# sapienta-ai/general-motion-retargeting

Measured on AMD Instinct MI355X. Metric: retargeted frames/sec (whole node) + max joint-angle err vs CPU ref, G1 29-DoF, higher is better.
Workload: dtype f64

## Files before the change

### __graft_entry__.py

```python
import os
import sys

ROOT = os.path.dirname(os.path.abspath(__file__))
if ROOT not in sys.path:
    sys.path.insert(0, ROOT)


def build() -> None:
    from general_motion_retargeting_amd import build as hip_build
    lib_path = hip_build.build(force=True)
    assert os.path.exists(lib_path)
    from oracle import oracle
    oracle.build(force=True)
    for p in list(hip_build.build_probe(force=True).values()) + list(hip_build.build_jlinv_probe(force=True).values()):
        assert os.path.exists(p)
    import general_motion_retargeting_amd as pkg
    from general_motion_retargeting_amd import _lib
    from general_motion_retargeting_amd.ik_config import pack_model, pack_taskset
    L = _lib.lib()
    for sym in _lib.EXPORTED_SYMBOLS:
        assert hasattr(L, sym), sym
    g = pkg.GeneralMotionRetargeting("smplx", "unitree_g1")
    oracle.check_abi(pack_model(g.model), pack_taskset(g.model, g._tables))


def smoke() -> None:
    import numpy as np
    import general_motion_retargeting_amd as pkg
    from general_motion_retargeting_amd import _lib, synth
    from oracle import oracle
    _lib.require_gpu()
    info = _lib.lib().gmr_backend_info().decode()
    g = pkg.GeneralMotionRetargeting("smplx", "unitree_g1", actual_human_height=1.75)
    human, q0 = synth.make_streams(g.model, g._tables, 4, 6, seed=0)
    q_hip, ns_hip, st = g.retarget_streams(human)
    q_cpu, ns_cpu, _ = oracle.retarget_streams(g._model_blob, g._taskset_blob, q0, human)
    assert (st == 0).all()
    assert np.array_equal(ns_hip, ns_cpu), "solver iteration counts differ"
    err = float(np.abs(q_hip - q_cpu).max())
    assert err < 1e-9, err
    for t, hd in enumerate(synth.streams_to_dicts(g._tables, human[0])):
        q = g.retarget(hd)
        assert np.abs(q - q_cpu[0, t]).max() < 1e-9
    km = pkg.KinematicsModel(g.xml_file)
    qq = q_hip[0]
    bp, br = km.forward_kinematics(qq[:, :3], qq[:, [4, 5, 6, 3]], qq[:, 7:])
    obp, obr = oracle.fk_f32(km._tree, qq[:, :3], qq[:, [4, 5, 6, 3]], qq[:, 7:])
    assert np.abs(bp - obp).max() < 5e-6 and np.abs(br - obr).max() < 5e-6
    print(f"smoke ok on {info}: max |q_hip - q_oracle| = {err:.2e}, solves/frame = {ns_hip.sum() / ns_hip[..., 0].size:.2f}")


if __name__ == "__main__":
    build()
    if len(sys.argv) > 1 and sys.argv[1] == "smoke":
        smoke()
```

### general_motion_retargeting_amd/build.py

```python
from __future__ import annotations

import hashlib
import os
import shutil
import subprocess
import sys

HERE = os.path.dirname(os.path.abspath(__file__))
CSRC = os.path.join(HERE, "csrc")
LIB = os.path.join(HERE, "libgmrhip.so")
OBJ = os.path.join(os.path.dirname(HERE), "build", "obj")
SOURCES = ["gmr_ik.hip", "gmr_ik_wide.hip", "gmr_fk.hip", "gmr_post.hip", "gmr_smplx.hip", "gmr_bvh.hip", "gmr_chunk.hip", "gmr_motion.hip", "gmr_body_state.hip", "gmr_tracker.hip", "gmr_tracker_links.hip", "gmr_tracker_preview.hip", "gmr_tracker_adaptive.hip", "gmr_tracker_anchor.hip", "gmr_tracker_control.hip", "gmr_comm.hip", "gmr_abi.hip"]
HEADERS = ["gmr_ik_wide_item.inc", "gmr_device_math.h", "gmr_ik_layout.h", "gmr_ik_wide_layout.h", "gmr_ik_prof.h", "gmr_ik_tree.h",
           "gmr_fk_tree.h", "gmr_fk_walk.h", "gmr_motion_sample.h", "gmr_philox.h", "gmr_tracker_dev.h", "gmr_link_plan.h", "gmr_handles.h", "gmr_post.h", "gmr_internal.h", "gmr_workspace.h", "../../include/gmr_hip.h", "../../include/gmr_types.h"]
FLAGS = ["-O3", "--offload-arch=gfx950", "-std=c++17", "-fPIC"]
PER_SOURCE_FLAGS = {"gmr_ik_wide.hip": ["-mllvm", "-disable-machine-licm", "-mllvm", "-sink-insts-to-avoid-spills=1"]}


def _hipcc() -> str:
    for c in (os.environ.get("HIPCC"), shutil.which("hipcc"), "/opt/rocm/bin/hipcc"):
        if c and os.path.exists(c):
            return c
    raise RuntimeError("hipcc not found (set HIPCC)")

# ... 11 lines not shown
    per_source = [] if os.environ.get("GMR_BUILD_NO_PER_SOURCE_FLAGS") else PER_SOURCE_FLAGS.get(src, [])
    defines = per_source + list(defines)
    tag = hashlib.sha1(" ".join(FLAGS + defines).encode()).hexdigest()[:10]
    obj = os.path.join(OBJ, f"{os.path.splitext(src)[0]}.{tag}.o")
    deps = [os.path.join(CSRC, src)] + [os.path.join(CSRC, h) for h in HEADERS]
    if force or verbose or not os.path.exists(obj) or any(os.path.getmtime(d) > os.path.getmtime(obj) for d in deps):
        cmd = [_hipcc()] + FLAGS + list(defines) + ["-c", os.path.join(CSRC, src), "-o", obj]
        if verbose:
            cmd.append("-Rpass-analysis=kernel-resource-usage")
        subprocess.check_call(cmd, cwd=CSRC)
    return obj


def _link(objs, out: str) -> str:
    subprocess.check_call([_hipcc(), "--offload-arch=gfx950", "-fPIC", "-shared", "-o", out + ".tmp"] + objs + ["-ldl"])
    os.replace(out + ".tmp", out)
    return out


def build(force: bool = False, verbose: bool = False) -> str:
    if not force and not needs_build():
        return LIB
    return _link([_object(s, [], force, verbose) for s in SOURCES], LIB)


PROBE_SRC = os.path.join(os.path.dirname(HERE), "tests", "hip", "math_probe.hip")
PROBE_LIBS = {"flags": os.path.join(os.path.dirname(PROBE_SRC), "libgmr_math_probe.so"),
              "wide": os.path.join(os.path.dirname(PROBE_SRC), "libgmr_math_probe_wide.so")}


def _build_probe_libs(src: str, libs: dict, force: bool) -> dict:
    deps = [src, os.path.join(CSRC, "gmr_device_math.h"), os.path.abspath(__file__)]
    extra = {"flags": [], "wide": PER_SOURCE_FLAGS["gmr_ik_wide.hip"]}
    for name, out in libs.items():
        if force or not os.path.exists(out) or any(os.path.getmtime(d) > os.path.getmtime(out) for d in deps):
            subprocess.check_call([_hipcc()] + FLAGS + extra[name] + ["-shared", "-o", out + ".tmp", src])
            os.replace(out + ".tmp", out)
    return dict(libs)


def build_probe(force: bool = False) -> dict:
    return _build_probe_libs(PROBE_SRC, PROBE_LIBS, force)


JLINV_PROBE_SRC = os.path.join(os.path.dirname(PROBE_SRC), "jlinv_apply_probe.hip")
JLINV_PROBE_LIBS = {"flags": os.path.join(os.path.dirname(PROBE_SRC), "libgmr_jlinv_apply_probe.so"),
                    "wide": os.path.join(os.path.dirname(PROBE_SRC), "libgmr_jlinv_apply_probe_wide.so")}


def build_jlinv_probe(force: bool = False) -> dict:
    return _build_probe_libs(JLINV_PROBE_SRC, JLINV_PROBE_LIBS, force)


def build_variant(name: str, defines=(), verbose: bool = False) -> str:
    out = os.path.join(HERE, f"libgmrhip_{name}.so")
    return _link([_object(s, list(defines), False, verbose) for s in SOURCES], out)


if __name__ == "__main__":
    if len(sys.argv) > 2 and sys.argv[1] == "--variant":
        print(build_variant(sys.argv[2], sys.argv[3:], verbose=False))
    else:
        print(build(force=True, verbose=True))
```

### general_motion_retargeting_amd/csrc/gmr_device_math.h

```cpp
#pragma once
#include <hip/hip_runtime.h>

namespace gmr {

struct d3 { double x, y, z; };
struct d4 { double w, x, y, z; };

__device__ __forceinline__ d3 operator+(d3 a, d3 b) { return {a.x + b.x, a.y + b.y, a.z + b.z}; }
__device__ __forceinline__ d3 operator-(d3 a, d3 b) { return {a.x - b.x, a.y - b.y, a.z - b.z}; }
__device__ __forceinline__ d3 operator*(double s, d3 a) { return {s * a.x, s * a.y, s * a.z}; }
__device__ __forceinline__ double dot(d3 a, d3 b) { return a.x * b.x + a.y * b.y + a.z * b.z; }
__device__ __forceinline__ d3 cross(d3 a, d3 b) {
  return {a.y * b.z - a.z * b.y, a.z * b.x - a.x * b.z, a.x * b.y - a.y * b.x};
}

__device__ __forceinline__ d4 qmul(d4 a, d4 b) {
  return {a.w * b.w - a.x * b.x - a.y * b.y - a.z * b.z,
          a.w * b.x + a.x * b.w + a.y * b.z - a.z * b.y,
          a.w * b.y - a.x * b.z + a.y * b.w + a.z * b.x,
          a.w * b.z + a.x * b.y - a.y * b.x + a.z * b.w};
}
__device__ __forceinline__ double fast_rsqrt(double x) {
  const double y = __builtin_amdgcn_rsq(x);
  const double e = fma(-x, y * y, 1.0);
// ... 284 lines not shown
  const d3 n = cross(w, rho), m = cross(w, n);
  const double k1 = (c1 + c2) * s;
  const d3 sq = {0.5 * rho.x - k1 * w.x - c2 * m.x, 0.5 * rho.y - k1 * w.y - c2 * m.y, 0.5 * rho.z - k1 * w.z - c2 * m.z};
  const double dq = -2.0 * c1 * s + 2.0 * c4 * s * t2, kw = -2.0 * c4 * s;
  const double da = 1.0 - a * t2;
  const d3 hw = {-0.5 * w.x, -0.5 * w.y, -0.5 * w.z};
  const double awj = a * dot(w, ej);
  const d3 hx = cross(hw, ej);
  const d3 v = {hx.x + awj * w.x + da * ej.x, hx.y + awj * w.y + da * ej.y, hx.z + awj * w.z + da * ej.z};
  const double wv = dot(w, v), rv = dot(rho, v);
  const double kr = c1 * wv, kq = c1 * rv + kw * wv;
  const d3 sx = cross(sq, v);
  const d3 y = {sx.x + kr * rho.x + kq * w.x + dq * v.x, sx.y + kr * rho.y + kq * w.y + dq * v.y, sx.z + kr * rho.z + kq * w.z + dq * v.z};
  const double awy = a * dot(w, y);
  const d3 hy = cross(hw, y);
  Ac[0] = v.x; Ac[1] = v.y; Ac[2] = v.z;
  Bc[0] = -(hy.x + awy * w.x + da * y.x); Bc[1] = -(hy.y + awy * w.y + da * y.y); Bc[2] = -(hy.z + awy * w.z + da * y.z);
}

__device__ __forceinline__ void se3_jlinv_coef5(const double e[6], const double aux[5], double coef[8]) {
  const d3 rho = {e[0], e[1], e[2]}, w = {e[3], e[4], e[5]};
  const double t2 = dot(w, w);
  coef[0] = 0.0; coef[1] = 1.0;
#pragma unroll
  for (int i = 2; i < 8; i++) coef[i] = 0.0;
  if (t2 < 1e-10) return;
  const double a = aux[0];
  double c1, c2, c3;
  if (t2 < 1e-2) {
    c1 = 1.0 / 6.0 - t2 / 120.0 + t2 * t2 / 5040.0 - t2 * t2 * t2 / 362880.0;
    c2 = -1.0 / 24.0 + t2 / 720.0 - t2 * t2 / 40320.0 + t2 * t2 * t2 / 3628800.0;
    c3 = -1.0 / 120.0 + t2 / 5040.0 - t2 * t2 / 362880.0 + t2 * t2 * t2 / 39916800.0;
  } else {
    const double t = aux[3], it = aux[4], sn = aux[1], cs = aux[2];
    const double it2 = it * it;
    c1 = (t - sn) * it2 * it;
    c2 = (1.0 - 0.5 * t2 - cs) * it2 * it2;
    c3 = (t - sn - t2 * t / 6.0) * it2 * it2 * it;
  }
  const double c4 = -0.5 * (c2 - 3.0 * c3);
  const double s = dot(w, rho);
  const d3 n = cross(w, rho), m = cross(w, n);
  const double k1 = (c1 + c2) * s;
  coef[0] = a;
  coef[1] = 1.0 - a * t2;
  coef[2] = c1;
  coef[3] = -2.0 * c4 * s;
  coef[4] = -2.0 * c1 * s + 2.0 * c4 * s * t2;
  coef[5] = 0.5 * rho.x - k1 * w.x - c2 * m.x;
  coef[6] = 0.5 * rho.y - k1 * w.y - c2 * m.y;
  coef[7] = 0.5 * rho.z - k1 * w.z - c2 * m.z;
}

__device__ __forceinline__ d3 jlinv_op_a(d3 w, d3 hw, double a, double da, d3 x) {
  const double aw = a * dot(w, x);
  const d3 hx = cross(hw, x);
  return d3{hx.x + aw * w.x + da * x.x, hx.y + aw * w.y + da * x.y, hx.z + aw * w.z + da * x.z};
}
__device__ __forceinline__ d3 jlinv_op_q(d3 w, d3 rho, d3 sq, double c1, double kw, double dq, d3 v) {
  const double wv = dot(w, v), rv = dot(rho, v);
  const double kr = c1 * wv, kq = c1 * rv + kw * wv;
  const d3 sx = cross(sq, v);
  return d3{sx.x + kr * rho.x + kq * w.x + dq * v.x, sx.y + kr * rho.y + kq * w.y + dq * v.y, sx.z + kr * rho.z + kq * w.z + dq * v.z};
}

__device__ __forceinline__ void se3_jlinv_apply5(const double e[6], const double coef[8], d3 jl, d3 ja, d3& top, d3& bot) {
  const d3 rho = {e[0], e[1], e[2]}, w = {e[3], e[4], e[5]};
  const double a = coef[0], da = coef[1], c1 = coef[2], kw = coef[3], dq = coef[4];
  const d3 sq = {coef[5], coef[6], coef[7]};
  const double h = a != 0.0 ? -0.5 : 0.0;
  const d3 hw = {h * w.x, h * w.y, h * w.z};
  const d3 v1 = jlinv_op_a(w, hw, a, da, ja);
  const d3 z = jlinv_op_a(w, hw, a, da, jlinv_op_q(w, rho, sq, c1, kw, dq, v1));
  const d3 u = jlinv_op_a(w, hw, a, da, jl);
  top = d3{z.x - u.x, z.y - u.y, z.z - u.z};
  bot = d3{-v1.x, -v1.y, -v1.z};
}

__device__ __forceinline__ int fresh_lane(int lane) {
#ifndef GMR_NO_FRESH_LANE
  asm volatile("" : "+v"(lane));
#endif
  return lane;
}

__device__ __forceinline__ double wave_sum(double v) {
#pragma unroll
  for (int off = 32; off > 0; off >>= 1) v += __shfl_xor(v, off, 64);
  return v;
}
__device__ __forceinline__ double wave_min(double v) {
#pragma unroll
  for (int off = 32; off > 0; off >>= 1) v = fmin(v, __shfl_xor(v, off, 64));
  return v;
}
__device__ __forceinline__ double wave_max(double v) {
#pragma unroll
  for (int off = 32; off > 0; off >>= 1) v = fmax(v, __shfl_xor(v, off, 64));
  return v;
}

__device__ __forceinline__ double dpp_row_shr(double v, double fill, int n) {
  union { double d; int i[2]; } a, f, r;
  a.d = v; f.d = fill;
  switch (n) {
    case 1: r.i[0] = __builtin_amdgcn_update_dpp(f.i[0], a.i[0], 0x111, 0xf, 0xf, false); r.i[1] = __builtin_amdgcn_update_dpp(f.i[1], a.i[1], 0x111, 0xf, 0xf, false); break;
// ... 63 lines not shown
```

### general_motion_retargeting_amd/csrc/gmr_ik.hip

```cpp
#include <hip/hip_runtime.h>
#include <math.h>
#include <stdint.h>

#include "../../include/gmr_hip.h"
#include "gmr_device_math.h"
#include "gmr_ik_layout.h"
#include "gmr_ik_prof.h"

namespace gmr {

template <int NW>
__device__ __forceinline__ void wsync() {
  if (NW == 1) __syncthreads();
  else __builtin_amdgcn_fence(__ATOMIC_SEQ_CST, "workgroup");
}
#define WSYNC() wsync<NW>()

#ifndef GMR_IK_MIN_WAVES
#define GMR_IK_MIN_WAVES 1
#endif
enum { QP_DENSE = 0, QP_TREE_SMALL = 1, QP_TREE = 2 };
enum { CMD_BUILD = 1, CMD_EXIT = 2, CMD_JBODY = 3 };

__device__ __forceinline__ double readlane_d(double v, int src) {
  int lo = __builtin_amdgcn_readlane(__double2loint(v), src);
  int hi = __builtin_amdgcn_readlane(__double2hiint(v), src);
  return __hiloint2double(hi, lo);
}

__device__ __forceinline__ double bpermute_d(int addr, double v) {
  int lo = __builtin_amdgcn_ds_bpermute(addr, __double2loint(v));
  int hi = __builtin_amdgcn_ds_bpermute(addr, __double2hiint(v));
  return __hiloint2double(hi, lo);
}

__device__ __forceinline__ double dot6(const double* a, const double* b) {
  return a[0] * b[0] + a[1] * b[1] + a[2] * b[2] + a[3] * b[3] + a[4] * b[4] + a[5] * b[5];
}

}
#include "gmr_ik_tree.h"
namespace gmr {

struct FkLane {
  int dep, hinge, src[IK_MAX_HOPS];
  d4 bq; d3 bp, ax;
};

template <class LT>
__device__ __forceinline__ FkLane fk_lane(const LT& L, const double* sm, const short* hop, const short* depth,
                                          const short* body_hinge, int lane) {
  FkLane F;
  const int b = lane < L.nb ? lane : 0;
  F.dep = lane < L.nb ? depth[b] : 0;
  F.hinge = lane < L.nb ? body_hinge[b] : -1;
#pragma unroll
  for (int r = 0; r < IK_MAX_HOPS; r++) F.src[r] = r < L.nhop ? 4 * hop[r * L.o.cap.nb + b] : 0;
  const double* bq = sm + L.o.body_quat + 4 * b;
  const double* bp = sm + L.o.body_pos + 3 * b;
  const double* ax = sm + L.o.axis + 3 * b;
  F.bq = d4{bq[0], bq[1], bq[2], bq[3]};
  F.bp = d3{bp[0], bp[1], bp[2]};
  F.ax = d3{ax[0], ax[1], ax[2]};
  return F;
}

template <int NW, class LT>
__device__ __forceinline__ void fk_wave(const LT& L, double* sm, const FkLane& F, int lane, Prof& pr) {
  lane = fresh_lane(lane);
  PROF_BEGIN(pr);
  const int nb = L.nb;
  double* q = sm + L.o.q;
  d3 pos = {0, 0, 0};
  d4 quat = {1, 0, 0, 0};
  const int dep = F.dep;
  if (lane < nb) {
    if (lane == 0) {
      quat = qnormalize(d4{q[3], q[4], q[5], q[6]});
      q[3] = quat.w; q[4] = quat.x; q[5] = quat.y; q[6] = quat.z;
      pos = d3{q[0], q[1], q[2]};
    } else {
      quat = F.bq;
      pos = F.bp;
      if (F.hinge >= 0) {
        const double* sc = sm + L.o.hsc + 2 * F.hinge;
        const double s = sc[0], c = sc[1];
        quat = qmul(quat, d4{c, F.ax.x * s, F.ax.y * s, F.ax.z * s});
      }
    }
  }
#pragma unroll
  for (int r = 0; r < IK_MAX_HOPS; r++) {
    if (r >= L.nhop) break;
    const int src = F.src[r];
    const d3 pa = {bpermute_d(src, pos.x), bpermute_d(src, pos.y), bpermute_d(src, pos.z)};
    const d4 qa = {bpermute_d(src, quat.w), bpermute_d(src, quat.x), bpermute_d(src, quat.y), bpermute_d(src, quat.z)};
    if (NW > 1) __builtin_amdgcn_s_waitcnt(0xc07f);
    if (lane < nb && dep >= (1 << r)) {
      pos = pa + qrot(qa, pos);
      quat = qmul(qa, quat);
    }
  }
  if (lane < nb) {
    quat = qnormalize(quat);
    double* o = sm + L.o.xa + 7 * lane;
    o[0] = pos.x; o[1] = pos.y; o[2] = pos.z; o[3] = quat.w; o[4] = quat.x; o[5] = quat.y; o[6] = quat.z;
    if (F.hinge >= 0) {
      d3 aw = qrot(quat, F.ax);
      double* xa = sm + L.o.xaxis + 3 * lane;
      xa[0] = aw.x; xa[1] = aw.y; xa[2] = aw.z;
    }
  }
  WSYNC();
  PROF_END(pr, PH_FK);
}

template <int NW, class LT>
__device__ __forceinline__ double errors_wave(const LT& L, double* sm, const short* task_body,
                                              const short* task_human, int K, int lane, Prof& pr) {
  lane = fresh_lane(lane);
  PROF_BEGIN(pr);
  double ss = 0.0;
  if (lane < K) {
    int b = task_body[lane], h = task_human[lane];
    const double* x = sm + L.o.xa + 7 * b;
    const double* tg = sm + L.o.tgt + 7 * h;
    double e[6], aux[5];
    se3_log_rel5(d3{x[0], x[1], x[2]}, d4{x[3], x[4], x[5], x[6]}, d3{tg[0], tg[1], tg[2]},
                 d4{tg[3], tg[4], tg[5], tg[6]}, e, aux);
    double* eo = sm + L.o.e + 6 * lane;
#pragma unroll
    for (int r = 0; r < 6; r++) { eo[r] = e[r]; ss += e[r] * e[r]; }
    double* ao = sm + L.o.eaux + 5 * lane;
#pragma unroll
    for (int r = 0; r < 5; r++) ao[r] = aux[r];
  }
  ss = row0_sum(ss);
  WSYNC();
  PROF_END(pr, PH_ERR);
  return sqrt(ss);
}

struct StageTabs {
  const short* task_body; const short* task_human; const short* pair_task; const short* pair_dof;
  const short* pair_index; const uint2* items;
};

template <int NW, class LT>
__device__ __forceinline__ double jlog_phase(const LT& L, double* sm, int stage, double lm_damping, int lane,
                                             Prof& pr) {
  lane = fresh_lane(lane);
  PROF_BEGIN(pr);
  const int K = L.K[stage];
  const double* wpos = sm + L.o.wpos[stage];
  const double* wrot = sm + L.o.wrot[stage];
  double mu = 0.0;
  const int k = lane & 15, j = lane >> 4;
  if (NW > 1) {
    if (lane < K) {
      const double* e = sm + L.o.e + 6 * lane;
      double ee[6];
#pragma unroll
      for (int r = 0; r < 6; r++) ee[r] = e[r];
      const double* ax = sm + L.o.eaux + 5 * lane;
      const double aux[5] = {ax[0], ax[1], ax[2], ax[3], ax[4]};
      double coef[8];
      se3_jlinv_coef5(ee, aux, coef);
      double* co = sm + L.o.M + 18 * lane;
#pragma unroll
      for (int r = 0; r < 8; r++) co[r] = coef[r];
      const double wp = wpos[lane], wr = wrot[lane];
      double* we = sm + L.o.we + 6 * lane;
#pragma unroll
      for (int r = 0; r < 6; r++) {
        double v = (r < 3 ? wp : wr) * ee[r];
        we[r] = v;
        mu += v * v;
      }
    }
  } else if (k < K && j < 3) {
    const double* e = sm + L.o.e + 6 * k;
    double ee[6];
#pragma unroll
    for (int r = 0; r < 6; r++) ee[r] = e[r];
    const double* ax = sm + L.o.eaux + 5 * k;
    const double aux[5] = {ax[0], ax[1], ax[2], ax[3], ax[4]};
    double Ac[3], Bc[3];
    se3_jlinv_col5(ee, aux, j, Ac, Bc);
    double* M = sm + L.o.M + 18 * k + j;
#pragma unroll
    for (int i = 0; i < 3; i++) { M[3 * i] = -Ac[i]; M[9 + 3 * i] = -Bc[i]; }
    if (j == 0) {
      double wp = wpos[k], wr = wrot[k];
      double* we = sm + L.o.we + 6 * k;
#pragma unroll
// ... 250 lines not shown
        item_store(Hb, w[k].y, acc, diag);
        acc = 0.0;
      }
    }
  }
}

template <int NW, class LT>
__device__ __forceinline__ void build_qp_main(const LT& L, double* sm, int stage, const StageTabs& tb,
                                              const short* hinge_body, const short* limited, int* ctl, int& epoch,
                                              double damping, double lm_damping, double limit_gain, int lane,
                                              int pk_main, Prof& pr) {
  double mu = jlog_phase<NW>(L, sm, stage, lm_damping, lane, pr);
  const double diag = damping + mu;
  if (NW == 1) {
    PROF_BEGIN(pr);
    pairs_phase(L, sm, stage, tb, hinge_body, lane, 64);
    WSYNC();
    PROF_END(pr, PH_PAIRS);
    PROF_BEGIN(pr);
    cvec_phase(L, sm, stage, tb, limited, limit_gain, lane);
    PROF_END(pr, PH_CVEC);
    PROF_BEGIN(pr);
    hacc_phase_g(L, sm, stage, tb.items, diag, lane);
    WSYNC();
    PROF_END(pr, PH_HACC);
  } else {
    PROF_BEGIN(pr);
    if (lane == 0) { int* c = ctl + 2 * (epoch & 1); c[0] = CMD_BUILD; c[1] = stage; (sm + L.o.scal)[0] = diag; }
    epoch++;
    __syncthreads();
    pairs_from_jbody(L, sm, stage, tb, lane, 64 * NW, nullptr, pk_main);
    __syncthreads();
    PROF_END(pr, PH_PAIRS);
    PROF_BEGIN(pr);
    cvec_phase(L, sm, stage, tb, limited, limit_gain, lane);
    PROF_END(pr, PH_CVEC);
    PROF_BEGIN(pr);
    __syncthreads();
    PROF_END(pr, PH_HACC);
  }
}

template <int NW, int QP, class LT>
__device__ __forceinline__ void helper_loop(const LT& L, double* sm, const uint32_t* sw, const short* si,
                                            const short* hinge_body, const int* ctl, int wave, int lane,
                                            Prof& hp) {
  TreeState bs = {0ull, 0ull};
  const TreeRows<16> rows_s = tree_rows<7, 9, false>(L, si, wave, lane);
  const TreeRows<18> rows_l = tree_rows<8, 10, false>(L, si, wave, lane);
  int pk[2];
#pragma unroll
  for (int st = 0; st < 2; st++) pk[st] = (unsigned short)(si + L.o.i_pair_task[st])[min(wave * 64 + lane, L.o.cap.p - 1)] & 15u;
  for (int epoch = 0;; epoch++) {
    PROF_BEGIN(hp);
    __syncthreads();
    PROF_END(hp, PH_PRE);
    const int cmd = ctl[2 * (epoch & 1)];
    if (cmd == CMD_EXIT) return;
    const int stage = ctl[2 * (epoch & 1) + 1];
    StageTabs tb = {si + L.o.i_task_body[stage], si + L.o.i_task_human[stage], si + L.o.i_pair_task[stage],
                    si + L.o.i_pair_dof[stage], si + L.o.i_pair_index[stage],
                    reinterpret_cast<const uint2*>(sw + L.w_items[stage])};
    if (cmd == CMD_JBODY) {
      PROF_BEGIN(hp);
      jbody_phase(L, sm, stage, tb, (wave - 1) * 64 + lane, 64 * (NW - 1));
      PROF_END(hp, PH_PAIRS);
      continue;
    }
    const double diag = (sm + L.o.scal)[0];
    uint2 first[4];
#pragma unroll
    for (int k = 0; k < 4; k++) first[k] = tb.items[k * L.nlanes + (wave - 1) * 64 + lane];
    PROF_BEGIN(hp);
    pairs_from_jbody(L, sm, stage, tb, wave * 64 + lane, 64 * NW, sw + L.o.w_zero + stage * IK_MAX_ZERO, pk[stage]);
    PROF_END(hp, PH_PAIRS);
    PROF_BEGIN(hp);
    __syncthreads();
    PROF_END(hp, PH_CVEC);
    PROF_BEGIN(hp);
    hacc_phase(L, sm, stage, tb, diag, (wave - 1) * 64 + lane, first);
    PROF_END(hp, PH_HACC);
    PROF_BEGIN(hp);
    __syncthreads();
    PROF_END(hp, PH_JLOG);
    if (QP == QP_TREE_SMALL) (void)solve_qp_tree<7, 9, false, true>(L, sm, const_cast<uint32_t*>(sw), si, wave, lane, bs, hp, rows_s);
    else (void)solve_qp_tree<8, 10, false, false>(L, sm, const_cast<uint32_t*>(sw), si, wave, lane, bs, hp, rows_l);
  }
}

template <int NVP, int NW, class LT>
__device__ __forceinline__ int solve_qp_regs(const LT& L, double* sm, int lane, int& st, Prof& pr) {
  constexpr int LDK = NVP + 1;
  const int n = L.nv, ldh = L.o.ldh;
  const double* H = sm + L.o.H;
  double* Kt = sm + L.o.Kt;
  const bool act = lane < n;
  const bool row = lane < NVP;
  const double lo = act ? (sm + L.o.lo)[lane] : 0.0, hi = act ? (sm + L.o.hi)[lane] : 0.0;
  const double ci = act ? (sm + L.o.c)[lane] : 0.0;
  const double* Hrow = H + (act ? lane : 0) * ldh;
  if (!act || (st < 0 && !(lo > -INFINITY)) || (st > 0 && !(hi < INFINITY))) st = 0;
  const double dual_tol = 1e-13 * (1.0 + rows3_max(fabs(ci)));
  const double ptol_lo = 1e-12 * (1.0 + fabs(lo)), ptol_hi = 1e-12 * (1.0 + fabs(hi));
  int pcount = 3, ninf_best = NVP + 1;
  for (int it = 0; it < 100; it++) {
    PROF_BEGIN(pr);
    PROF_COUNT(pr, PH_NFACT);
    const unsigned long long fixedm = __ballot(act && st != 0);
    const double xfix = st < 0 ? lo : (st > 0 ? hi : 0.0);
    double rhs = act ? (st != 0 ? xfix : -ci) : 0.0;
    {
      unsigned long long m = fixedm;
      while (m) {
        int j = __ffsll((long long)m) - 1;
        m &= m - 1;
// ... 62 lines not shown
    double x = b;
    WSYNC();
    PROF_END(pr, PH_SUBST);
    PROF_BEGIN(pr);
    double g = 0.0;
    if (fixedm) {
      g = ci;
#pragma unroll
      for (int j = 0; j < NVP; j++) {
        double xj = readlane_d(x, j);
        if (j < n) g += (act ? Hrow[j] : 0.0) * xj;
      }
    }
    int newst = st;
    bool viol = false;
    if (act) {
      if (st == 0) {
        if (x < lo - ptol_lo) { viol = true; newst = -1; }
        else if (x > hi + ptol_hi) { viol = true; newst = 1; }
      } else if (st < 0) {
        if (g < -dual_tol) { viol = true; newst = 0; }
      } else {
        if (g > dual_tol) { viol = true; newst = 0; }
      }
    }
    const unsigned long long vm = __ballot(viol);
    PROF_END(pr, PH_MULT);
    if (vm == 0ull) {
      if (act) (sm + L.o.x)[lane] = fmin(fmax(x, lo), hi);
      WSYNC();
      return GMR_STATUS_OK;
    }
    const int ninf = __popcll(vm);
    if (ninf < ninf_best) { ninf_best = ninf; pcount = 3; st = newst; }
    else if (pcount > 0) { pcount--; st = newst; }
    else {
      int top = 63 - __clzll((long long)vm);
      if (lane == top) st = newst;
    }
  }
  return GMR_STATUS_QP_MAXITER;
}

template <class LT>
__device__ __forceinline__ void hinge_sincos(const LT& L, double* sm, int lane) {
  if (lane >= 6 && lane < L.nv) {
    double s, c;
    sincos_small(0.5 * (sm + L.o.q)[7 + lane - 6], &s, &c);
    double* sc = sm + L.o.hsc + 2 * (lane - 6);
    sc[0] = s; sc[1] = c;
  }
}

template <int NW, class LT>
__device__ __forceinline__ void integrate_wave(const LT& L, double* sm, double dt, int lane, Prof& pr) {
  lane = fresh_lane(lane);
  PROF_BEGIN(pr);
  double* q = sm + L.o.q;
  const double* dq = sm + L.o.x;
  const bool base = lane == 0, hinge = lane >= 6 && lane < L.nv;
  double half = 0.0, inv = 0.0;
  bool rotate = false;
  if (base) {
    q[0] += dq[0]; q[1] += dq[1]; q[2] += dq[2];
    const double n2 = dq[3] * dq[3] + dq[4] * dq[4] + dq[5] * dq[5];
    rotate = n2 >= 1e-30 * dt * dt;
    if (rotate) { inv = fast_rsqrt(n2); half = 0.5 * (n2 * inv); }
  } else if (hinge) {
    const double th = q[7 + lane - 6] + dq[lane];
    q[7 + lane - 6] = th;
    half = 0.5 * th;
  }
  double s, c;
  sincos_small(half, &s, &c);
  if (base) {
    d4 quat = qnormalize(d4{q[3], q[4], q[5], q[6]});
    if (rotate) quat = qmul(quat, d4{c, dq[3] * inv * s, dq[4] * inv * s, dq[5] * inv * s});
    q[3] = quat.w; q[4] = quat.x; q[5] = quat.y; q[6] = quat.z;
  } else if (hinge) {
    double* sc = sm + L.o.hsc + 2 * (lane - 6);
    sc[0] = s; sc[1] = c;
  }
  WSYNC();
  PROF_END(pr, PH_INTEG);
}

template <int NW, class LT>
__device__ __forceinline__ void preprocess_wave(const LT& L, double* sm, const short* is_foot, int human_root,
                                                double ground_offset, int flags, int lane, Prof& pr) {
  lane = fresh_lane(lane);
  PROF_BEGIN(pr);
  const double* raw = sm + L.o.raw;
  double* tgt = sm + L.o.tgt;
  double z = INFINITY;
  d3 p = {0, 0, 0};
  d4 uq = {1, 0, 0, 0};
  const bool on = lane < L.nhum;
  if (on) {
    const double* in = raw + 7 * lane;
    const double* rp = raw + 7 * human_root;
    const double* sc = sm + L.o.scale;
    double sr = sc[human_root];
    d3 srp = {sr * rp[0], sr * rp[1], sr * rp[2]};
    if (lane == human_root) p = srp;
    else {
      double s = sc[lane];
      p = d3{(in[0] - rp[0]) * s + srp.x, (in[1] - rp[1]) * s + srp.y, (in[2] - rp[2]) * s + srp.z};
    }
    const double* qo = sm + L.o.quat_off + 4 * lane;
    const double* po = sm + L.o.pos_off + 3 * lane;
    d4 q = qnormalize(d4{in[3], in[4], in[5], in[6]});
    uq = qnormalize(qmul(q, qnormalize(d4{qo[0], qo[1], qo[2], qo[3]})));
    p = p + qrot(uq, d3{po[0], po[1], po[2]});
    if (is_foot[lane] && p.x == p.x) z = p.z;
  }
  if (flags & GMR_FLAG_OFFSET_TO_GROUND) {
    double lowest = row0_min(z);
    p.z = p.z - lowest + ground_offset;
  }
  if (on) {
    double* o = tgt + 7 * lane;
    o[0] = p.x; o[1] = p.y; o[2] = p.z; o[3] = uq.w; o[4] = uq.x; o[5] = uq.y; o[6] = uq.z;
  }
  WSYNC();
  PROF_END(pr, PH_PRE);
}

template <int NVP, int NW, int QP>
__global__ __launch_bounds__(64 * NW, GMR_IK_MIN_WAVES) void ik_streams_kernel(const uint4* __restrict__ image, IkLay<NVP, NW> L, IkParams P,
                                                             int S, int T, const double* __restrict__ q0,
// ... 3 lines not shown
                                                             int32_t* __restrict__ nsolve,
                                                             int32_t* __restrict__ status,
                                                             double* __restrict__ tgt_out,
                                                             double* __restrict__ err_out,
                                                             unsigned long long* __restrict__ prof_out) {
  extern __shared__ __align__(16) double smem[];
  const int wave = threadIdx.x >> 6;
  const int lane = threadIdx.x & 63;
  const int s = blockIdx.x;
  if (s >= S) return;
  double* sm = smem;
  Prof pr;
#ifdef GMR_IK_PROFILE
  for (int i = 0; i < PH_COUNT; i++) pr.acc[i] = 0;
  const unsigned long long k_t0 = __builtin_amdgcn_s_memtime(), k_r0 = __builtin_amdgcn_s_memrealtime();
#endif
  short* si = reinterpret_cast<short*>(smem + L.o.n_double);
  uint32_t* sw = reinterpret_cast<uint32_t*>(si + L.o.n_short);
  int* ctl = reinterpret_cast<int*>(sw + L.o.w_ctl);
  short* hop = si + L.o.i_hop;
  short* depth = si + L.o.i_depth;
  short* body_hinge = si + L.o.i_body_hinge;
  short* hinge_body = si + L.o.i_hinge_body;
  short* limited = si + L.o.i_limited;
  short* is_foot = si + L.o.i_is_foot;

  const int nv = L.nv, nq = L.nq, nhum = L.nhum;
  {
    uint4* dst = reinterpret_cast<uint4*>(smem);
    const int n16 = (L.smem_bytes + 15) >> 4;
    for (int i = threadIdx.x; i < n16; i += 64 * NW) dst[i] = image[i];
  }
  __syncthreads();
  if (NW > 1 && wave > 0) {
    helper_loop<NW, QP>(L, sm, sw, si, hinge_body, ctl, wave, lane, pr);
#ifdef GMR_IK_PROFILE
    if (wave == 1 && lane == 0 && prof_out)
      for (int i = 0; i < PH_COUNT; i++) prof_out[((size_t)S + s) * PH_COUNT + i] = pr.acc[i];
#endif
    return;
  }
  const double* prm = sm + L.o.params;
  const int max_iter = P.max_iter, human_root = P.human_root;
  const int use0 = P.use0, use1 = P.use1;

  for (int i = lane; i < nq; i += 64) (sm + L.o.q)[i] = q0[(size_t)s * nq + i];
  WSYNC();
  hinge_sincos(L, sm, lane);
  WSYNC();
  const FkLane fkc = fk_lane(L, sm, hop, depth, body_hinge, lane);
  int pk_main[2];
#pragma unroll
  for (int st = 0; st < 2; st++) pk_main[st] = (unsigned short)(si + L.o.i_pair_task[st])[lane] & 15u;
  fk_wave<NW>(L, sm, fkc, lane, pr);

  const int Ts = len ? min(len[s], T) : T;
  const size_t fstride = (size_t)nhum * 7;
  const double* hs = human + (size_t)s * T * fstride;
  int stat = GMR_STATUS_OK;
  int qp_state = 0;
  TreeState tree_state = {0ull, 0ull};
  const TreeRows<16> rows_s = (NW > 1 && QP == QP_TREE_SMALL) ? tree_rows<7, 9, false>(L, si, 0, lane) : TreeRows<16>{};
  const TreeRows<18> rows_l = (NW > 1 && QP != QP_TREE_SMALL) ? tree_rows<8, 10, false>(L, si, 0, lane) : TreeRows<18>{};
  const TreeRows<16> rows_r = (NW == 1 && QP == QP_TREE_SMALL) ? tree_rows<7, 9, true>(L, si, 0, lane) : TreeRows<16>{};
  int h_stage = -1;
  int epoch = 0;
  double r0 = 0.0, r1 = 0.0;
  if (Ts > 0) {
    if (lane < (int)fstride) r0 = hs[lane];
    if (lane + 64 < (int)fstride) r1 = hs[lane + 64];
  }
  for (int t = 0; t < Ts; t++) {
    if (lane < (int)fstride) (sm + L.o.raw)[lane] = r0;
    if (lane + 64 < (int)fstride) (sm + L.o.raw)[lane + 64] = r1;
    if (t + 1 < Ts) {
      const double* nx = hs + (size_t)(t + 1) * fstride;
      if (lane < (int)fstride) r0 = nx[lane];
      if (lane + 64 < (int)fstride) r1 = nx[lane + 64];
    }
    WSYNC();
    int ns0 = 0, ns1 = 0;
    const size_t f = (size_t)s * T + t;
    if (stat == GMR_STATUS_OK) {
      preprocess_wave<NW>(L, sm, is_foot, human_root, prm[4], flags, lane, pr);
      if (tgt_out)
        for (int i = lane; i < (int)fstride; i += 64) tgt_out[f * fstride + i] = (sm + L.o.tgt)[i];
      double last_E = -1.0;
      for (int stage = 0; stage < 2; stage++) {
        if (!(stage == 0 ? use0 : use1) || (flags & GMR_FLAG_EVAL_ONLY)) continue;
        const StageTabs tb = {si + L.o.i_task_body[stage], si + L.o.i_task_human[stage], si + L.o.i_pair_task[stage],
                              si + L.o.i_pair_dof[stage], si + L.o.i_pair_index[stage],
                              reinterpret_cast<const uint2*>(NW == 1 ? reinterpret_cast<const uint32_t*>(image) + L.g_items[stage]
                                                                     : sw + L.w_items[stage])};
        const int K = L.K[stage];
        if (h_stage != stage) {
          for (int i = lane; i < nv * L.o.ldh; i += 64) (sm + L.o.H)[i] = 0.0;
          h_stage = stage;
          WSYNC();
        }
        if (NW > 1 && !(stage == 1 && (use1 & 4) && last_E >= 0.0)) {
          if (lane == 0) { int* c = ctl + 2 * (epoch & 1); c[0] = CMD_JBODY; c[1] = stage; }
          epoch++;
          __syncthreads();
        }
        double curr = (stage == 1 && (use1 & 2) && last_E >= 0.0) ? last_E
                                                                 : errors_wave<NW>(L, sm, tb.task_body, tb.task_human, K, lane, pr);
        int nsol = 0, num_iter = 0;
        for (;;) {
          build_qp_main<NW>(L, sm, stage, tb, hinge_body, limited, ctl, epoch, prm[0], prm[1], prm[3], lane, pk_main[stage], pr);
          PROF_COUNT(pr, PH_NSOLVE);
          int rc;
          if (NW > 1) {
            rc = QP == QP_TREE_SMALL ? solve_qp_tree<7, 9, false, true>(L, sm, sw, si, 0, lane, tree_state, pr, rows_s)
                                     : solve_qp_tree<8, 10, false, false>(L, sm, sw, si, 0, lane, tree_state, pr, rows_l);
          } else if (QP == QP_TREE_SMALL) {
            rc = solve_qp_tree<7, 9, true, true>(L, sm, sw, si, 0, lane, tree_state, pr, rows_r);
          } else {
            rc = solve_qp_regs<NVP, NW>(L, sm, lane, qp_state, pr);
          }
          if (rc != GMR_STATUS_OK) { stat = rc; break; }
          integrate_wave<NW>(L, sm, prm[5], lane, pr);
          fk_wave<NW>(L, sm, fkc, lane, pr);
          if (NW > 1) {
            if (lane == 0) { int* c = ctl + 2 * (epoch & 1); c[0] = CMD_JBODY; c[1] = stage; }
            epoch++;
            __syncthreads();
          }
          double next = errors_wave<NW>(L, sm, tb.task_body, tb.task_human, K, lane, pr);
          last_E = next;
          nsol++;
          if (nsol > 1) num_iter++;
          if (!(curr - next > prm[2] && num_iter < max_iter)) break;
          curr = next;
        }
        if (stage == 0) ns0 = nsol; else ns1 = nsol;
        if (stat != GMR_STATUS_OK) break;
      }
    }
    if (err_out && stat == GMR_STATUS_OK) {
      for (int stage = 0; stage < 2; stage++) {
        double E = 0.0;
        if (stage == 0 ? use0 : use1)
          E = errors_wave<NW>(L, sm, si + L.o.i_task_body[stage], si + L.o.i_task_human[stage], L.K[stage], lane, pr);
        if (lane == 0) err_out[2 * f + stage] = E;
      }
    }
    for (int i = lane; i < nq; i += 64) q_out[f * nq + i] = (sm + L.o.q)[i];
    if (lane == 0) { nsolve[2 * f] = ns0; nsolve[2 * f + 1] = ns1; }
    WSYNC();
  }
  if (lane == 0) status[s] = stat;
  if (NW > 1) {
    if (lane == 0) ctl[2 * (epoch & 1)] = CMD_EXIT;
    __syncthreads();
  }
#ifdef GMR_IK_PROFILE
  pr.acc[PH_TICKS] = __builtin_amdgcn_s_memtime() - k_t0;
  pr.acc[PH_REALTIME] = __builtin_amdgcn_s_memrealtime() - k_r0;
  if (lane == 0 && prof_out)
    for (int i = 0; i < PH_COUNT; i++) prof_out[(size_t)s * PH_COUNT + i] = pr.acc[i];
#else
  (void)prof_out;
#endif
}

}

template <int NVP, int NW, int QP>
static hipError_t launch_nvp(const uint4* d_image, const gmr::IkLayout* L, const gmr::IkParams* P, int S, int T,
                             const double* d_q0, const double* d_human,
                             const int32_t* d_len, int flags, double* d_q_out, int32_t* d_nsolve, int32_t* d_status,
                             double* d_tgt_out, double* d_err_out, hipStream_t stream, unsigned long long* d_prof) {
  hipLaunchKernelGGL((gmr::ik_streams_kernel<NVP, NW, QP>), dim3(S), dim3(64 * NW), L->smem_bytes, stream, d_image,
                     gmr::IkLay<NVP, NW>(static_cast<const gmr::IkDims&>(*L)), *P, S, T, d_q0, d_human, d_len, flags, d_q_out, d_nsolve, d_status,
                     d_tgt_out, d_err_out, d_prof);
  return hipGetLastError();
}

#define GMR_ARGS d_image, L, P, S, T, d_q0, d_human, d_len, flags, d_q_out, d_nsolve, d_status, d_tgt_out, d_err_out, stream, d_prof
#define GMR_DISPATCH(NVP_)                                                                             \
  case NVP_:                                                                                           \
    if (L->nw == 1) return L->tree_small ? launch_nvp<NVP_, 1, gmr::QP_TREE_SMALL>(GMR_ARGS)           \
                                         : launch_nvp<NVP_, 1, gmr::QP_DENSE>(GMR_ARGS);               \
    return L->tree_small ? launch_nvp<NVP_, 4, gmr::QP_TREE_SMALL>(GMR_ARGS)                           \
                         : launch_nvp<NVP_, 4, gmr::QP_TREE>(GMR_ARGS);

extern "C" hipError_t gmr_launch_ik_streams(const uint4* d_image, const gmr::IkLayout* L, const gmr::IkParams* P,
                                            int S, int T, const double* d_q0, const double* d_human,
                                            const int32_t* d_len, int flags, double* d_q_out, int32_t* d_nsolve,
                                            int32_t* d_status, double* d_tgt_out, double* d_err_out,
                                            hipStream_t stream, unsigned long long* d_prof) {
  if (S <= 0 || T <= 0) return hipSuccess;
  switch (L->nvp) {
    GMR_DISPATCH(28)
    GMR_DISPATCH(32)
    GMR_DISPATCH(36)
    GMR_DISPATCH(48)
    default: return hipErrorInvalidValue;
  }
}

template <int NVP>
static const void* kernel_of(int nw, int tree_small) {
  if (nw == 1) return tree_small ? reinterpret_cast<const void*>(gmr::ik_streams_kernel<NVP, 1, gmr::QP_TREE_SMALL>)
                                 : reinterpret_cast<const void*>(gmr::ik_streams_kernel<NVP, 1, gmr::QP_DENSE>);
  return tree_small ? reinterpret_cast<const void*>(gmr::ik_streams_kernel<NVP, 4, gmr::QP_TREE_SMALL>)
                    : reinterpret_cast<const void*>(gmr::ik_streams_kernel<NVP, 4, gmr::QP_TREE>);
}

extern "C" hipError_t gmr_ik_set_max_smem(int nvp, int nw, int tree_small, int bytes) {
  const void* f = nullptr;
  switch (nvp) {
    case 28: f = kernel_of<28>(nw, tree_small); break;
    case 32: f = kernel_of<32>(nw, tree_small); break;
    case 36: f = kernel_of<36>(nw, tree_small); break;
    case 48: f = kernel_of<48>(nw, tree_small); break;
    default: return hipErrorInvalidValue;
  }
  return hipFuncSetAttribute(f, hipFuncAttributeMaxDynamicSharedMemorySize, bytes);
}
```

### general_motion_retargeting_amd/csrc/gmr_ik_prof.h

```cpp
#pragma once
#include <hip/hip_runtime.h>

namespace gmr {

enum { PH_PRE, PH_FK, PH_ERR, PH_JLOG, PH_PAIRS, PH_CVEC, PH_HACC, PH_KBUILD, PH_CHOL, PH_SUBST, PH_RATIO,
       PH_MULT, PH_INTEG, PH_IO, PH_NFACT, PH_NSOLVE, PH_TICKS, PH_REALTIME, PH_COUNT };
#ifdef GMR_IK_PROFILE
struct Prof {
  unsigned long long acc[PH_COUNT];
  unsigned long long t0;
  __device__ __forceinline__ void begin() { t0 = __builtin_amdgcn_s_memtime(); }
  __device__ __forceinline__ void end(int ph) { acc[ph] += __builtin_amdgcn_s_memtime() - t0; }
  __device__ __forceinline__ void count(int ph) { acc[ph] += 1; }
};
#define PROF_BEGIN(p) (p).begin()
#define PROF_END(p, ph) (p).end(ph)
#define PROF_COUNT(p, ph) (p).count(ph)
#else
struct Prof {};
#define PROF_BEGIN(p)
#define PROF_END(p, ph)
#define PROF_COUNT(p, ph)
#endif

}
```

Baseline: 843,900.

## Split FK and error evaluation across waves to overlap position FK with rotation log

In the multi-wave IK kernel, the main wave now normalizes the base quaternion during integration, then signals helper wave 1 to run position forward kinematics. Meanwhile the main wave computes body orientations with its own quaternion-only walk and evaluates the rotational half of the SE3 log error. After a barrier it finishes the translational half using the helper's positions, and the helper waves go straight into the Jacobian body phase. This is meant to take the serial FK-then-error chain off the main wave's critical path, at the cost of duplicated quaternion work, an extra barrier, and reordered floating-point steps that could move results away from the CPU reference.

Measured after the change: 862,900 (median of 6 runs). 1.02x the previous value.

```diff
diff --git a/__graft_entry__.py b/__graft_entry__.py
--- a/__graft_entry__.py
+++ b/__graft_entry__.py
@@ -12,7 +12,8 @@
     assert os.path.exists(lib_path)
     from oracle import oracle
     oracle.build(force=True)
-    for p in list(hip_build.build_probe(force=True).values()) + list(hip_build.build_jlinv_probe(force=True).values()):
+    for p in (list(hip_build.build_probe(force=True).values()) + list(hip_build.build_jlinv_probe(force=True).values())
+              + [hip_build.build_split_probe(force=True)]):
         assert os.path.exists(p)
     import general_motion_retargeting_amd as pkg
     from general_motion_retargeting_amd import _lib
diff --git a/general_motion_retargeting_amd/build.py b/general_motion_retargeting_amd/build.py
--- a/general_motion_retargeting_amd/build.py
+++ b/general_motion_retargeting_amd/build.py
@@ -87,6 +87,19 @@
     return _build_probe_libs(JLINV_PROBE_SRC, JLINV_PROBE_LIBS, force)
 
 
+SPLIT_PROBE_SRC = os.path.join(os.path.dirname(PROBE_SRC), "split_eval_probe.hip")
+SPLIT_PROBE_LIB = os.path.join(os.path.dirname(PROBE_SRC), "libgmr_split_eval_probe.so")
+
+
+def build_split_probe(force: bool = False) -> str:
+    deps = [SPLIT_PROBE_SRC, os.path.abspath(__file__)] + [os.path.join(CSRC, h) for h in ["gmr_ik.hip"] + HEADERS]
+    out = SPLIT_PROBE_LIB
+    if force or not os.path.exists(out) or any(os.path.getmtime(d) > os.path.getmtime(out) for d in deps):
+        subprocess.check_call([_hipcc()] + FLAGS + ["-shared", "-o", out + ".tmp", SPLIT_PROBE_SRC])
+        os.replace(out + ".tmp", out)
+    return out
+
+
 def build_variant(name: str, defines=(), verbose: bool = False) -> str:
     out = os.path.join(HERE, f"libgmrhip_{name}.so")
     return _link([_object(s, list(defines), False, verbose) for s in SOURCES], out)
diff --git a/general_motion_retargeting_amd/csrc/gmr_device_math.h b/general_motion_retargeting_amd/csrc/gmr_device_math.h
--- a/general_motion_retargeting_amd/csrc/gmr_device_math.h
+++ b/general_motion_retargeting_amd/csrc/gmr_device_math.h
@@ -360,6 +360,52 @@
   coef[7] = 0.5 * rho.z - k1 * w.z - c2 * m.z;
 }
 
+
+__device__ __forceinline__ void se3_log_rel5_rot(d4 qb, d4 qt, double w3[3], double aux[5]) {
+  const d4 q = qmul(qconj(qb), qt);
+  const double n2 = q.x * q.x + q.y * q.y + q.z * q.z;
+  const double cw = fabs(q.w);
+  double f, sh = 0.0, ch = 1.0, inv_sh = 0.0, half = 0.0;
+  if (n2 < 1e-10) {
+    f = 2.0 / q.w - 2.0 / 3.0 * n2 / (q.w * q.w * q.w);
+  } else {
+    const double inv_n = fast_rsqrt(n2);
+    sh = n2 * inv_n; ch = cw; inv_sh = inv_n;
+    half = atan2_q1(sh, ch);
+    bool neg = q.w < 0.0;
+    if (cw < 1e-10) {
+      half = 1.57079632679489661923; sh = 1.0; ch = 6.123233995736766e-17; inv_sh = 1.0;
+      neg = !(q.w > 0.0);
+    }
+    f = 2.0 * half * inv_n;
+    if (neg) f = -f;
+  }
+  const d3 w = {f * q.x, f * q.y, f * q.z};
+  const double t2 = dot(w, w);
+  double a;
+  if (t2 < 1e-2) {
+    aux[1] = 0.0; aux[2] = 1.0; aux[3] = 0.0; aux[4] = 0.0;
+    a = 1.0 / 12.0 + t2 * (1.0 / 720.0 + t2 * (1.0 / 30240.0 + t2 * (1.0 / 1209600.0 + t2 / 47900160.0)));
+  } else {
+    const double t = 2.0 * half, inv_t = fast_rcp(t);
+    aux[1] = 2.0 * sh * ch;
+    aux[2] = 1.0 - 2.0 * sh * sh;
+    aux[3] = t; aux[4] = inv_t;
+    a = (sh - half * ch) * inv_sh * (inv_t * inv_t);
+  }
+  aux[0] = a;
+  w3[0] = w.x; w3[1] = w.y; w3[2] = w.z;
+}
+
+__device__ __forceinline__ void se3_log_rel5_pos(d3 pb, d4 qb, d3 pt, const double w3[3], double a, double v3[3]) {
+  const d3 pbt = qrot_inv(qb, pt - pb);
+  const d3 w = {w3[0], w3[1], w3[2]};
+  const d3 wp = cross(w, pbt);
+  const d3 wwp = cross(w, wp);
+  const d3 v = pbt - 0.5 * wp + a * wwp;
+  v3[0] = v.x; v3[1] = v.y; v3[2] = v.z;
+}
+
 __device__ __forceinline__ d3 jlinv_op_a(d3 w, d3 hw, double a, double da, d3 x) {
   const double aw = a * dot(w, x);
   const d3 hx = cross(hw, x);
diff --git a/general_motion_retargeting_amd/csrc/gmr_ik.hip b/general_motion_retargeting_amd/csrc/gmr_ik.hip
--- a/general_motion_retargeting_amd/csrc/gmr_ik.hip
+++ b/general_motion_retargeting_amd/csrc/gmr_ik.hip
@@ -20,7 +20,7 @@
 #define GMR_IK_MIN_WAVES 1
 #endif
 enum { QP_DENSE = 0, QP_TREE_SMALL = 1, QP_TREE = 2 };
-enum { CMD_BUILD = 1, CMD_EXIT = 2, CMD_JBODY = 3 };
+enum { CMD_BUILD = 1, CMD_EXIT = 2, CMD_JBODY = 3, CMD_FK = 4 };
 
 __device__ __forceinline__ double readlane_d(double v, int src) {
   int lo = __builtin_amdgcn_readlane(__double2loint(v), src);
@@ -65,7 +65,7 @@
   return F;
 }
 
-template <int NW, class LT>
+template <int NW, bool NORM = true, class LT>
 __device__ __forceinline__ void fk_wave(const LT& L, double* sm, const FkLane& F, int lane, Prof& pr) {
   lane = fresh_lane(lane);
   PROF_BEGIN(pr);
@@ -76,8 +76,11 @@
   const int dep = F.dep;
   if (lane < nb) {
     if (lane == 0) {
-      quat = qnormalize(d4{q[3], q[4], q[5], q[6]});
-      q[3] = quat.w; q[4] = quat.x; q[5] = quat.y; q[6] = quat.z;
+      quat = d4{q[3], q[4], q[5], q[6]};
+      if (NORM) {
+        quat = qnormalize(quat);
+        q[3] = quat.w; q[4] = quat.x; q[5] = quat.y; q[6] = quat.z;
+      }
       pos = d3{q[0], q[1], q[2]};
     } else {
       quat = F.bq;
@@ -141,6 +144,89 @@
   return sqrt(ss);
 }
 
+struct RotHalf { d4 qb; double w[3], a; };
+
+template <class LT>
+__device__ __forceinline__ d4 qwalk_wave(const LT& L, const double* sm, const FkLane& F, int lane) {
+  const int nb = L.nb;
+  const double* q = sm + L.o.q;
+  d4 quat = {1, 0, 0, 0};
+  const int dep = F.dep;
+  if (lane < nb) {
+    if (lane == 0) {
+      quat = d4{q[3], q[4], q[5], q[6]};
+    } else {
+      quat = F.bq;
+      if (F.hinge >= 0) {
+        const double* sc = sm + L.o.hsc + 2 * F.hinge;
+        const double s = sc[0], c = sc[1];
+        quat = qmul(quat, d4{c, F.ax.x * s, F.ax.y * s, F.ax.z * s});
+      }
+    }
+  }
+#pragma unroll
+  for (int r = 0; r < IK_MAX_HOPS; r++) {
+    if (r >= L.nhop) break;
+    const int src = F.src[r];
+    const d4 qa = {bpermute_d(src, quat.w), bpermute_d(src, quat.x), bpermute_d(src, quat.y), bpermute_d(src, quat.z)};
+    __builtin_amdgcn_s_waitcnt(0xc07f);
+    if (lane < nb && dep >= (1 << r)) quat = qmul(qa, quat);
+  }
+  if (lane < nb) quat = qnormalize(quat);
+  return quat;
+}
+
+template <class LT>
+__device__ __forceinline__ RotHalf rot_half_wave(const LT& L, double* sm, const FkLane& F, int tq, int th, int K, int lane, Prof& pr) {
+  lane = fresh_lane(lane);
+  PROF_BEGIN(pr);
+  const d4 quat = qwalk_wave(L, sm, F, lane);
+  RotHalf R;
+  R.qb = d4{bpermute_d(tq, quat.w), bpermute_d(tq, quat.x), bpermute_d(tq, quat.y), bpermute_d(tq, quat.z)};
+  R.w[0] = R.w[1] = R.w[2] = 0.0; R.a = 0.0;
+  PROF_END(pr, PH_QWALK);
+  PROF_BEGIN(pr);
+  if (lane < K) {
+    const double* tg = sm + L.o.tgt + th;
+    double aux[5];
+    se3_log_rel5_rot(R.qb, d4{tg[3], tg[4], tg[5], tg[6]}, R.w, aux);
+    R.a = aux[0];
+    double* eo = sm + L.o.e + 6 * lane;
+#pragma unroll
+    for (int r = 0; r < 3; r++) eo[3 + r] = R.w[r];
+    double* ao = sm + L.o.eaux + 5 * lane;
+#pragma unroll
+    for (int r = 0; r < 5; r++) ao[r] = aux[r];
+  }
+  PROF_END(pr, PH_ROT);
+  return R;
+}
+
+template <class LT>
+__device__ __forceinline__ double pos_half_wave(const LT& L, double* sm, const RotHalf& R, int tq, int th, int K, int lane, Prof& pr) {
+  lane = fresh_lane(lane);
+  PROF_BEGIN(pr);
+  double ss = 0.0;
+  if (lane < K) {
+    const double* x = sm + L.o.xa + 7 * (tq >> 2);
+    const double* tg = sm + L.o.tgt + th;
+    double v[3];
+    se3_log_rel5_pos(d3{x[0], x[1], x[2]}, R.qb, d3{tg[0], tg[1], tg[2]}, R.w, R.a, v);
+    double* eo = sm + L.o.e + 6 * lane;
+#pragma unroll
+    for (int r = 0; r < 3; r++) { eo[r] = v[r]; ss += v[r] * v[r]; }
+#pragma unroll
+    for (int r = 0; r < 3; r++) ss += R.w[r] * R.w[r];
+  }
+  ss = row0_sum(ss);
+  __builtin_amdgcn_fence(__ATOMIC_SEQ_CST, "workgroup");
+  PROF_END(pr, PH_POS);
+  return sqrt(ss);
+}
+
+#ifdef GMR_IK_WALKS_ONLY
+}
+#else
 struct StageTabs {
   const short* task_body; const short* task_human; const short* pair_task; const short* pair_dof;
   const short* pair_index; const uint2* items;
@@ -497,6 +583,7 @@
   int pk[2];
 #pragma unroll
   for (int st = 0; st < 2; st++) pk[st] = (unsigned short)(si + L.o.i_pair_task[st])[min(wave * 64 + lane, L.o.cap.p - 1)] & 15u;
+  const FkLane fkc = fk_lane(L, sm, si + L.o.i_hop, si + L.o.i_depth, si + L.o.i_body_hinge, lane);
   for (int epoch = 0;; epoch++) {
     PROF_BEGIN(hp);
     __syncthreads();
@@ -507,6 +594,16 @@
     StageTabs tb = {si + L.o.i_task_body[stage], si + L.o.i_task_human[stage], si + L.o.i_pair_task[stage],
                     si + L.o.i_pair_dof[stage], si + L.o.i_pair_index[stage],
                     reinterpret_cast<const uint2*>(sw + L.w_items[stage])};
+    if (cmd == CMD_FK) {
+      if (wave == 1) fk_wave<NW, false>(L, sm, fkc, lane, hp);
+      PROF_BEGIN(hp);
+      __syncthreads();
+      PROF_END(hp, PH_ERR);
+      PROF_BEGIN(hp);
+      jbody_phase(L, sm, stage, tb, (wave - 1) * 64 + lane, 64 * (NW - 1));
+      PROF_END(hp, PH_PAIRS);
+      continue;
+    }
     if (cmd == CMD_JBODY) {
       PROF_BEGIN(hp);
       jbody_phase(L, sm, stage, tb, (wave - 1) * 64 + lane, 64 * (NW - 1));
@@ -675,7 +772,7 @@
   }
 }
 
-template <int NW, class LT>
+template <int NW, bool NORM = false, class LT>
 __device__ __forceinline__ void integrate_wave(const LT& L, double* sm, double dt, int lane, Prof& pr) {
   lane = fresh_lane(lane);
   PROF_BEGIN(pr);
@@ -699,6 +796,7 @@
   if (base) {
     d4 quat = qnormalize(d4{q[3], q[4], q[5], q[6]});
     if (rotate) quat = qmul(quat, d4{c, dq[3] * inv * s, dq[4] * inv * s, dq[5] * inv * s});
+    if (NORM) quat = qnormalize(quat);
     q[3] = quat.w; q[4] = quat.x; q[5] = quat.y; q[6] = quat.z;
   } else if (hinge) {
     double* sc = sm + L.o.hsc + 2 * (lane - 6);
@@ -808,6 +906,13 @@
   int pk_main[2];
 #pragma unroll
   for (int st = 0; st < 2; st++) pk_main[st] = (unsigned short)(si + L.o.i_pair_task[st])[lane] & 15u;
+  int tq_main[2], th_main[2];
+#pragma unroll
+  for (int st = 0; st < 2; st++) {
+    const bool on = NW > 1 && lane < L.K[st];
+    tq_main[st] = on ? 4 * (si + L.o.i_task_body[st])[lane] : 0;
+    th_main[st] = on ? 7 * (si + L.o.i_task_human[st])[lane] : 0;
+  }
   fk_wave<NW>(L, sm, fkc, lane, pr);
 
   const int Ts = len ? min(len[s], T) : T;
@@ -875,14 +980,22 @@
             rc = solve_qp_regs<NVP, NW>(L, sm, lane, qp_state, pr);
           }
           if (rc != GMR_STATUS_OK) { stat = rc; break; }
-          integrate_wave<NW>(L, sm, prm[5], lane, pr);
-          fk_wave<NW>(L, sm, fkc, lane, pr);
+          double next;
           if (NW > 1) {
-            if (lane == 0) { int* c = ctl + 2 * (epoch & 1); c[0] = CMD_JBODY; c[1] = stage; }
+            integrate_wave<NW, true>(L, sm, prm[5], lane, pr);
+            if (lane == 0) { int* c = ctl + 2 * (epoch & 1); c[0] = CMD_FK; c[1] = stage; }
             epoch++;
             __syncthreads();
+            const RotHalf rh = rot_half_wave(L, sm, fkc, tq_main[stage], th_main[stage], K, lane, pr);
+            PROF_BEGIN(pr);
+            __syncthreads();
+            PROF_END(pr, PH_K2);
+            next = pos_half_wave(L, sm, rh, tq_main[stage], th_main[stage], K, lane, pr);
+          } else {
+            integrate_wave<NW>(L, sm, prm[5], lane, pr);
+            fk_wave<NW>(L, sm, fkc, lane, pr);
+            next = errors_wave<NW>(L, sm, tb.task_body, tb.task_human, K, lane, pr);
           }
-          double next = errors_wave<NW>(L, sm, tb.task_body, tb.task_human, K, lane, pr);
           last_E = next;
           nsol++;
           if (nsol > 1) num_iter++;
@@ -975,3 +1088,4 @@
   }
   return hipFuncSetAttribute(f, hipFuncAttributeMaxDynamicSharedMemorySize, bytes);
 }
+#endif
diff --git a/general_motion_retargeting_amd/csrc/gmr_ik_prof.h b/general_motion_retargeting_amd/csrc/gmr_ik_prof.h
--- a/general_motion_retargeting_amd/csrc/gmr_ik_prof.h
+++ b/general_motion_retargeting_amd/csrc/gmr_ik_prof.h
@@ -4,7 +4,10 @@
 namespace gmr {
 
 enum { PH_PRE, PH_FK, PH_ERR, PH_JLOG, PH_PAIRS, PH_CVEC, PH_HACC, PH_KBUILD, PH_CHOL, PH_SUBST, PH_RATIO,
-       PH_MULT, PH_INTEG, PH_IO, PH_NFACT, PH_NSOLVE, PH_TICKS, PH_REALTIME, PH_COUNT };
+       PH_MULT, PH_INTEG, PH_IO,
+       PH_QWALK, PH_ROT, PH_K2, PH_POS,
+       PH_NFACT, PH_NSOLVE, PH_TICKS, PH_REALTIME, PH_COUNT };
+enum { PH_NTIME = PH_NFACT };
 #ifdef GMR_IK_PROFILE
 struct Prof {
   unsigned long long acc[PH_COUNT];
```
